# Mingtzge/PVE-MCC_for_unsignalized_intersection

Measured on AMD Instinct MI355X. Metric: env-steps/sec (vehicles x envs x steps/s) at 128 veh x 4096 envs, higher is better.
Workload: dtype f64

## Files before the change

pve-mcc_for_unsignalized_intersection_amd/csrc/pve_hip.hip:

```cpp
#include <hip/hip_runtime.h>
#include <mutex>
#include <new>

#include "pve_host.h"
#include "pve_tick_core.h"
#include "pve_tick_geo.h"
#include "pve_actor.h"

using namespace pve;

#ifdef PVE_AB_KNOBS
#define PVE_KNOB(name_) getenv(name_)
#else
#define PVE_KNOB(name_) ((const char *)nullptr)
#endif
#ifndef PVE_HOME_DEFAULT
#define PVE_HOME_DEFAULT 1
#endif

typedef __attribute__((address_space(4))) const char *KernargPtr;
#define PVE_PHASE_MARK(idx)                                                              \
    if (P.phase_cycles) {                                                                \
        unsigned long long now_ = wall_clock64();                                        \
        pc_[idx] = now_ - tprev_;                                                        \
        tprev_ = now_;                                                                   \
    }

__device__ __forceinline__ void lds_barrier() { __syncthreads(); }
template <int CAP>
__global__ __launch_bounds__(CAP) __attribute__((amdgpu_waves_per_eu(CAP == 128 ? 5 : 4, CAP == 128 ? 5 : 4))) void k_tick(const Const c_arg, const Params P_arg)
{
    KernargPtr ka0_ = (KernargPtr)__builtin_amdgcn_kernarg_segment_ptr();
    const PVE_AS4 Const &c = *(const PVE_AS4 Const *)ka0_;
    const PVE_AS4 Params &P = *(const PVE_AS4 Params *)(ka0_ + ((sizeof(Const) + 7) / 8 * 8));
    typedef Shared<CAP, false> ShT;
    __shared__ ShT sh;
    const int t = threadIdx.x;
    const int env = blockIdx.x;
    Regs r;
    typedef Tick<CAP, ShT> T;
    unsigned long long pc_[12] = {0, 0, 0, 0, 0, 0, 0, 0, 0, 0, 0, 0};
    unsigned long long tprev_ = P.phase_cycles ? wall_clock64() : 0ull;
    T::ph_load(c, P, env, t, sh, r);
    lds_barrier();
    PVE_PHASE_MARK(0)
    if (P.stop_phase == 0) return;
    T::ph_step1(c, P, env, t, sh, r);
    lds_barrier();
    PVE_PHASE_MARK(1)
    if (P.stop_phase == 1) return;
    T::ph_step2(c, t, sh, r);
    T::ph_lists_a(c, t, sh);
    lds_barrier();
    PVE_PHASE_MARK(2)
    if (P.stop_phase == 2) return;
    T::ph_step3(c, t, sh, r);
    T::ph_step3_publish(t, sh, r);
    T::ph_lists_b(t, sh);
    lds_barrier();
    PVE_PHASE_MARK(3)
    if (P.stop_phase == 3) return;
    T::ph_build(c, t, sh, r);
    lds_barrier();
    PVE_PHASE_MARK(4)
    if (P.stop_phase == 4) return;
    T::ph_rank(t, sh, env);
    lds_barrier();
    PVE_PHASE_MARK(5)
    if (P.stop_phase == 5) return;
    T::ph_scan(c, t, sh, r);
    PVE_PHASE_MARK(11)
    T::ph_reward(c, t, sh, r);
    lds_barrier();
    PVE_PHASE_MARK(6)
    if (P.stop_phase == 6) return;
    T::ph_effects(c, t, sh, r);
    lds_barrier();
    PVE_PHASE_MARK(7)
    if (P.stop_phase == 7) return;
    T::ph_prefetch_arrival(P, env, t, sh, r, NL);
    T::ph_lock(c, t, sh, r);
    lds_barrier();
    T::ph_lock2(t, sh, r);
    lds_barrier();
    PVE_PHASE_MARK(8)
    if (P.stop_phase == 8) return;
    T::ph_final(c, P, env, t, sh, r);
    PVE_PHASE_MARK(9)
    if (P.out.state_pre) {
        __threadfence_block();
        __syncthreads();
        if constexpr (CAP <= 128) {
            T::ph_state_publish(P.out, t, sh, r);
            __syncthreads();
            T::ph_state_coop(P, P.out, env, t, sh);
        } else T::ph_state(P, env, t, sh, r);
        PVE_PHASE_MARK(10)
    }
    if (P.phase_cycles && (t & 63) == 0) {
        unsigned long long *row = P.phase_cycles + ((size_t)env * (CAP / 64) + (t >> 6)) * 16;
#pragma unroll
        for (int k = 0; k < 12; k++) row[k] += pc_[k];
    }
}

template <int CAP>
__device__ __forceinline__ void rollout_actor(const unsigned char *packed, const float *aprm, double *act, const slot_t<CAP> *adsts,
                                              int n_ctl, const void *rows, bool obs_f32, size_t base, int t)
{
    const pve_v8h *A1 = (const pve_v8h *)(packed + AP_A1), *A2 = (const pve_v8h *)(packed + AP_A2);
    const int lane = t & 63, hf = lane >> 5, j = lane & 31;
    for (int tile = t >> 6; 32 * tile < n_ctl; tile += CAP / 64) {
        const int slot = adsts[32 * tile + j];
        const int srow = slot == SLOT_NONE<CAP> ? 0 : slot;
        float x[16];
        if (obs_f32) actor_fetch_env((const float *)rows + base * OBSW, srow, hf, x);
        else actor_fetch_env((const double *)rows + base * OBSW, srow, hf, x);
        const float a = actor_tile32(A1, A2, aprm, x, lane);
        if (lane < 32 && slot != SLOT_NONE<CAP>) act[slot] = (double)a;
    }
}

__device__ __forceinline__ void rollout_noise(const PVE_AS4 RolloutArgsNoisy &R, int env, int tick, Regs &r)
{
    const double sigma = R.noise.sigma;
    if (__builtin_expect(sigma != 0, 0)) {
        if (r.alive && (r.meta & M_CONTROL))
            r.act = r.act + sigma * action_noise_z(R.noise.seed, (int64_t)env + R.noise.env_offset, r.id, R.noise.tick0 + (uint32_t)tick);
    }
}

__device__ __forceinline__ double table_action(const double *table, int row, int table_ids, int id)
{
    const unsigned col = (unsigned)id < (unsigned)table_ids ? (unsigned)id : (unsigned)(table_ids - 1);
    return *(const double *)((const char *)(table + (size_t)row * (size_t)table_ids) + col * 8u);
}

#ifdef PVE_QUEUE_TRACE
#define Q_TRACE(R_) ((R_).q_trace)
#else
#define Q_TRACE(R_) ((unsigned long long *)nullptr)
#endif
__device__ __forceinline__ unsigned q_xcc_id()
{
    return __builtin_amdgcn_s_getreg((3 << 11) | (0 << 6) | 20) & 0xFu;
}
__device__ __forceinline__ unsigned q_load(const unsigned *p) { return __hip_atomic_load(p, __ATOMIC_RELAXED, __HIP_MEMORY_SCOPE_AGENT); }
__device__ __forceinline__ void q_store(unsigned *p, unsigned v) { __hip_atomic_store(p, v, __ATOMIC_RELAXED, __HIP_MEMORY_SCOPE_AGENT); }
__device__ __forceinline__ void q_dequeue(RolloutQueue *Q, int n_shards, int n_envs, int n_chunks, unsigned xcc, int &shard, int &probe,
                                          int &env, int &chunk)
{
    for (;;) {
        if (shard >= 0) {
            const unsigned es = (unsigned)(n_envs - shard + n_shards - 1) / (unsigned)n_shards;
            const unsigned i = __hip_atomic_fetch_add(&Q->s[shard].head, 1u, __ATOMIC_RELAXED, __HIP_MEMORY_SCOPE_AGENT);
            if (i < es * (unsigned)n_chunks) {
                const unsigned c = i / es;
                env = shard + (int)(i - c * es) * n_shards; chunk = (int)c;
                return;
            }
        }
        shard = -1;
        while (probe < n_shards) {
            const int cand = (int)((xcc + (unsigned)probe) % (unsigned)n_shards);
            probe++;
            if (cand >= n_envs) continue;
            unsigned seen = q_load(&Q->s[cand].owner);
            if (seen == 0u)
                __hip_atomic_compare_exchange_strong(&Q->s[cand].owner, &seen, xcc + 1u, __ATOMIC_RELAXED, __ATOMIC_RELAXED, __HIP_MEMORY_SCOPE_AGENT);
            if (seen != 0u && seen != xcc + 1u) continue;
            const unsigned es = (unsigned)(n_envs - cand + n_shards - 1) / (unsigned)n_shards;
            if (q_load(&Q->s[cand].head) >= es * (unsigned)n_chunks) continue;
            shard = cand;
            break;
        }
        if (shard < 0) { env = -1; chunk = 0; return; }
    }
}

__device__ __forceinline__ bool q_take(const PVE_AS4 RolloutArgs &R, int n_envs, int t0, int *q_word, int &env, int &chunk, int &k_base,
                                       int &n_ticks)
{
    RolloutQueue *Q = (RolloutQueue *)R.queue;
    unsigned *done = R.queue + sizeof(RolloutQueue) / 4;
    if (t0 == 0) {
        int shard = q_word[2], probe = q_word[3], e, ch;
        const unsigned long long tq0 = Q_TRACE(R) ? wall_clock64() : 0ull;
        q_dequeue(Q, R.n_shards, n_envs, R.n_full + R.n_taper, q_xcc_id(), shard, probe, e, ch);
        q_word[0] = e; q_word[1] = ch; q_word[2] = shard; q_word[3] = probe;
        const unsigned long long tq1 = Q_TRACE(R) ? wall_clock64() : 0ull;
        if (e >= 0)
            while ((int)(q_load(&done[e]) - (R.done_base + (unsigned)ch)) < 0) __builtin_amdgcn_s_sleep(8);
        if (Q_TRACE(R) && e >= 0) {
            unsigned long long *row = Q_TRACE(R) + ((size_t)ch * n_envs + e) * 8;
            row[0] = tq0; row[1] = tq1; row[2] = wall_clock64();
            row[6] = (unsigned long long)blockIdx.x | ((unsigned long long)q_xcc_id() << 32);
        }
    }
    __syncthreads();
    env = __builtin_amdgcn_readfirstlane(q_word[0]);
    chunk = __builtin_amdgcn_readfirstlane(q_word[1]);
    if (env < 0) return false;
    rollout_item(R, chunk, k_base, n_ticks);
    return true;
}
__device__ __forceinline__ void q_publish(const PVE_AS4 RolloutArgs &R, int n_envs, int t0, int env, int chunk)
{
    const unsigned long long tf0 = (Q_TRACE(R) && t0 == 0) ? wall_clock64() : 0ull;
    asm volatile("s_waitcnt vmcnt(0)" ::: "memory");
    __syncthreads();
    if (t0 == 0) q_store(R.queue + sizeof(RolloutQueue) / 4 + env, R.done_base + (unsigned)chunk + 1u);
    if (Q_TRACE(R) && t0 == 0) {
        unsigned long long *row = Q_TRACE(R) + ((size_t)chunk * n_envs + env) * 8;
        row[4] = tf0; row[5] = wall_clock64();
    }
}
__device__ __forceinline__ void q_leave(const PVE_AS4 RolloutArgs &R, int t0)
{
    RolloutQueue *Q = (RolloutQueue *)R.queue;
    if (t0 == 0) {
        const unsigned left = __hip_atomic_fetch_add(&Q->exits, 1u, __ATOMIC_RELAXED, __HIP_MEMORY_SCOPE_AGENT);
        if (left + 1u == gridDim.x) {
            for (int k = 0; k < QUEUE_MAX_SHARDS; k++) { q_store(&Q->s[k].head, 0u); q_store(&Q->s[k].owner, 0u); }
            q_store(&Q->exits, 0u);
        }
    }
}

template <int CAP, int WPE, bool PROF = false, bool ACT = false, bool TRAIN = false, bool IDT = false, bool PERS = false>
__global__ __launch_bounds__(CAP) __attribute__((amdgpu_waves_per_eu(WPE, WPE))) void k_rollout(const Const c_arg, const Params P_arg,
                                                                                               const typename rollout_args<ACT>::type R_arg)
{
    typedef typename rollout_args<ACT>::type RArgs;
    static_assert(!PERS || !PROF, "the persistent form has no phase-cycle diagnostics variant");
    static_assert(!(ACT && IDT), "one action source per variant");
    KernargPtr ka0_ = (KernargPtr)__builtin_amdgcn_kernarg_segment_ptr();
    constexpr size_t OFF_P = (sizeof(Const) + 7) / 8 * 8, OFF_R = OFF_P + (sizeof(Params) + 7) / 8 * 8;
    typedef Shared<CAP, (CAP == 128 && WPE == 4), (WPE == 5)> ShT;
    __shared__ ShT sh;
    __shared__ __attribute__((aligned(64))) float aprm[ACT ? PV_TOTAL : 1];
    __shared__ slot_t<CAP> adsts[ACT ? CAP : 1];
    __shared__ int q_word[4];
    int adst = -1;
    int t0_ = threadIdx.x;
    int env0_ = PERS ? 0 : blockIdx.x;
    int k_base_ = 0, chunk_ = 0;
    bool aprm_staged = false;
    if (CAP > 64) { if (__builtin_amdgcn_readfirstlane(t0_) < 64) __builtin_amdgcn_s_setprio(3); else if (WPE == 5) __builtin_amdgcn_s_setprio(2); }
    KernargPtr kav_ = ka0_;
    Regs r;
    FinCarry fc;
    typedef Tick<CAP, ShT> T;
    unsigned long long pc_[12] = {0, 0, 0, 0, 0, 0, 0, 0, 0, 0, 0, 0};
    unsigned long long tprev_ = PROF ? wall_clock64() : 0ull;
    const unsigned long long sclk0_ = PROF ? clock64() : 0ull, wclk0_ = tprev_;
#undef PVE_PHASE_MARK
#define PVE_PHASE_MARK(idx)                                                              \
    if (PROF) {                                                                          \
        unsigned long long now_ = wall_clock64();                                        \
        pc_[idx] += now_ - tprev_;                                                       \
        tprev_ = now_;                                                                   \
    }
    int pool_idx, n_ticks;
    if constexpr (PERS) { if (t0_ == 0) { q_word[2] = -1; q_word[3] = 0; } }
  for (;;) {
    {
        const PVE_AS4 Const &c = *(const PVE_AS4 Const *)ka0_;
        const PVE_AS4 Params &P = *(const PVE_AS4 Params *)(ka0_ + OFF_P);
        const PVE_AS4 RArgs &R = *(const PVE_AS4 RArgs *)(ka0_ + OFF_R);
        pool_idx = R.pool_tick0;
        n_ticks = R.n_ticks;
        const double *act0 = nullptr;
        if constexpr (PERS) {
            int e, ch, kb, nt;
            if (!q_take(R, P.n_envs, t0_, q_word, e, ch, kb, nt)) break;
            env0_ = e; chunk_ = ch; k_base_ = kb; n_ticks = nt;
            if (R.source == 1 || R.source == 3) pool_idx = (R.pool_tick0 + k_base_) % R.n_pool;
            if (R.source == 1) act0 = R.pool + (size_t)pool_idx * (size_t)P.n_envs * CAP;
        }
        bool act_handed = false;
        if constexpr (PERS && ACT) {
            act_handed = chunk_ > 0;
            if (act_handed) act0 = R.actor_actions;
        }
        if constexpr (ACT) if (!act_handed) {
            if (!PERS || !aprm_staged) {
                const float *gp = (const float *)(R.actor_packed + AP_PRM);
                for (int n = t0_; n < PV_TOTAL; n += CAP) aprm[n] = gp[n];
            }
            const int mt = P.i32[I_META][(size_t)env0_ * CAP + t0_];
            const bool cc = (mt & (M_ALIVE | M_CONTROL)) == (M_ALIVE | M_CONTROL);
            vote<CAP / 64>(sh.m_ctl, t0_, cc);
            adsts[t0_] = (slot_t<CAP>)SLOT_NONE<CAP>;
            lds_barrier();
            if (cc) adsts[mask_rank<CAP / 64>(sh.m_ctl, t0_)] = (slot_t<CAP>)t0_;
            const int nc = mask_count<CAP / 64>(sh.m_ctl);
            lds_barrier();
            rollout_actor<CAP>(R.actor_packed, aprm, sh.act_next, adsts, nc, R.actor_obs, P.obs_f32 != 0, (size_t)env0_ * CAP, t0_);
            lds_barrier();
        }
        if constexpr (PERS && ACT) {
            if (!aprm_staged && act_handed) {
                const float *gp = (const float *)(R.actor_packed + AP_PRM);
                for (int n = t0_; n < PV_TOTAL; n += CAP) aprm[n] = gp[n];
            }
            aprm_staged = true;
        }
        if constexpr (PERS) {
            T::template ph_load<true, ACT>(c, P, env0_, t0_, sh, r, act0, true);
            if (Q_TRACE(R) && t0_ == 0) Q_TRACE(R)[((size_t)chunk_ * P.n_envs + env0_) * 8 + 3] = wall_clock64();
        } else T::ph_load(c, P, env0_, t0_, sh, r);
        if constexpr (ACT) { if (!act_handed) r.act = sh.act_next[t0_]; }
        if constexpr (IDT) {
            r.act = r.alive ? table_action(R.pool, pool_idx, R.table_ids, r.id) : 0.0;
        }
        T::ph_home_store(t0_, sh, r);
    }
    double sp_act = 0;
    for (int k = 0; k < n_ticks; k++) {
        if constexpr (PERS) env0_ = __builtin_amdgcn_readfirstlane(env0_);
        asm volatile("" : "+s"(kav_), "+v"(t0_), "+s"(env0_));
        const KernargPtr ka = kav_;
        const int t = t0_, env = env0_;
#ifndef PVE_NO_RANGE_ASSUME
#ifdef PVE_ASSUME_ONE_WAVE_ONLY
        if constexpr (CAP == 64)
#endif
        __builtin_assume(t >= 0 && t < CAP);
#endif
        const PVE_AS4 Const &c = *(const PVE_AS4 Const *)ka;
        const PVE_AS4 Params &P = *(const PVE_AS4 Params *)(ka + OFF_P);
        const PVE_AS4 RArgs &R = *(const PVE_AS4 RArgs *)(ka + OFF_R);
        lds_barrier();
        PVE_PHASE_MARK(0)
        if constexpr (CAP == 64 && !PERS) {
            const int na = __builtin_amdgcn_readfirstlane(sh.hd.n_alive);
#ifndef PVE_NO_LOAD_PRIO
            if (na > 38) __builtin_amdgcn_s_setprio(3);
            else if (na > 32) __builtin_amdgcn_s_setprio(2);
            else if (na > 26) __builtin_amdgcn_s_setprio(1);
            else __builtin_amdgcn_s_setprio(0);
#endif
        }
        if (k > 0) T::ph_tick_init(c, t, sh, r);
        if constexpr (ACT) rollout_noise(R, env, k_base_ + k, r);
        T::ph_step1(c, P, env, t, sh, r);
        lds_barrier();
        PVE_PHASE_MARK(1)
        T::ph_step2(c, t, sh, r);
        T::ph_lists_a(c, t, sh);
        lds_barrier();
        PVE_PHASE_MARK(2)
        const bool last_tick = k + 1 == n_ticks;
        T::ph_step3(c, t, sh, r, last_tick);
        T::ph_step3_publish(t, sh, r);
        T::ph_lists_b(t, sh);
        lds_barrier();
        PVE_PHASE_MARK(3)
        if constexpr (ShT::HOME) {
            T::ph_build_prep(c, t, sh, r);
            T::ph_scan_init(r);
            if (__builtin_amdgcn_readfirstlane((int)sh.loff[NL]) <= ShT::POOL) {
                T::template ph_build_fill<false>(c, t, sh, r, 0, NL);
                lds_barrier();
                T::template ph_rank<false>(t, sh);
                lds_barrier();
                T::template ph_scan_lists<false>(c, t, sh, r, 0, NL);
            } else
            for (int d0 = 0, pass = 0; d0 < NL; pass++) {
                const int d1 = __builtin_amdgcn_readfirstlane(T::group_end(sh, d0));
                T::template ph_build_fill<true>(c, t, sh, r, d0, d1);
                lds_barrier();
                T::template ph_rank<true>(t, sh, pass, d0, d1);
                lds_barrier();
                T::template ph_scan_lists<true>(c, t, sh, r, d0, d1);
                d0 = d1;
                if (d0 < NL) lds_barrier();
            }
        } else {
        T::ph_build(c, t, sh, r);
        lds_barrier();
        PVE_PHASE_MARK(4)
        T::ph_rank(t, sh);
        lds_barrier();
        PVE_PHASE_MARK(5)
        T::ph_scan(c, t, sh, r);
        }
        PVE_PHASE_MARK(11)
        T::ph_reward(c, t, sh, r);
        lds_barrier();
        PVE_PHASE_MARK(6)
        int nx = -1;
        if (k + 1 < n_ticks) { pool_idx = (pool_idx + 1 == R.n_pool) ? 0 : pool_idx + 1; nx = pool_idx; }
        if constexpr (IDT) {
            int my_id = r.id;
            if constexpr (ShT::HOME) my_id = sh.h_id[t];
            r.act_nx = (nx >= 0 && r.alive) ? table_action(R.pool, nx, R.table_ids, my_id) : 0.0;
        } else T::ph_prefetch_action(P, R, env, t, nx, r);
        T::ph_effects(c, t, sh, r);
        lds_barrier();
        PVE_PHASE_MARK(7)
        T::ph_prefetch_arrival(P, env, t, sh, r, NL);
        bool sp_late = false;
        if constexpr (IDT) {
            const unsigned want = (unsigned)(sh.m_spawn[0] & 0xFFFull);
            sp_late = __builtin_popcount(want) > CAP - sh.hd.n_alive;
            sp_act = 0;
            if (t < NL && nx >= 0 && !sp_late && ((want >> t) & 1u))
                sp_act = table_action(R.pool, nx, R.table_ids, sh.hd.id_seq + __builtin_popcount(want & ((1u << t) - 1u)));
        }
        T::ph_lock(c, t, sh, r, last_tick);
        lds_barrier();
        T::ph_lock2(t, sh, r, last_tick);
        T::ph_keep_prefix(t, sh);
        lds_barrier();
        PVE_PHASE_MARK(8)
        if constexpr (!ACT && !IDT) { if (!(ShT::HOME && last_tick)) T::ph_park_action(t, sh, r); }
        const Outputs O = T::template tick_outputs<TRAIN>(P, R, k_base_ + k);
        if constexpr (ACT) {
            adst = -1;
            T::template ph_final<true>(c, P, O, env, t, sh, r, fc, true, &adst);
            adsts[t] = (slot_t<CAP>)(adst < 0 ? SLOT_NONE<CAP> : adst);
        } else T::template ph_final<true, !TRAIN>(c, P, O, env, t, sh, r, fc, k + 1 == n_ticks || (TRAIN && O.state_pre != nullptr));
        PVE_PHASE_MARK(9)
        if constexpr (IDT) {
            if (fc.new_slot >= 0) sh.act_next[fc.new_slot] = r.act_nx;
            if (sp_late) sp_act = (fc.sp_slot >= 0 && nx >= 0) ? table_action(R.pool, nx, R.table_ids, fc.sp_id) : 0.0;
        }
        HomeRegs hr;
        T::ph_home_take(t, sh, r, fc, hr);
        if (fc.still) {
            T::ph_stage_header(t, sh, fc);
            T::ph_carry_over(t, sh, r, fc);
        } else {
            lds_barrier();
            if constexpr (TRAIN) {
                if (O.state_pre) {
                    if constexpr (CAP <= 128) {
                        T::ph_state_publish(O, t, sh, r);
                        lds_barrier();
                        T::template ph_state_coop<PERS>(P, O, env, t, sh);
                    } else T::template ph_state<PERS>(P, O, env, t, sh, r);
                }
            }
            T::ph_stage(c, t, sh, r, fc);
            T::ph_home_put(t, sh, fc, hr);
            if constexpr (IDT) { if (fc.sp_slot >= 0) sh.act_next[fc.sp_slot] = sp_act; }
            if constexpr (ACT) {
                if (fc.sp_slot >= 0) sh.act_next[fc.sp_slot] = (double)aprm[PV_A0];
                const bool hand_on = PERS && k + 1 == n_ticks && chunk_ + 1 < R.n_full + R.n_taper;
                if (k + 1 < n_ticks || hand_on)
                    rollout_actor<CAP>(R.actor_packed, aprm, sh.act_next, adsts, fc.n_ctl, O.obs_post, P.obs_f32 != 0,
                                       (size_t)env * CAP, t);
                if (hand_on) {
                    lds_barrier();
                    R.actor_actions[(size_t)env * CAP + t] = sh.act_next[t];
                }
            }
            lds_barrier();
            if (k + 1 < n_ticks) T::ph_reload(t, sh, r);
        }
        PVE_PHASE_MARK(10)
    }
    {
        const PVE_AS4 Params &P = *(const PVE_AS4 Params *)(ka0_ + OFF_P);
        T::ph_flush(P, env0_, t0_, sh);
        if (PROF && P.phase_cycles && (t0_ & 63) == 0) {
            unsigned long long *row = P.phase_cycles + ((size_t)env0_ * (CAP / 64) + (t0_ >> 6)) * 16;
#pragma unroll
            for (int k = 0; k < 12; k++) row[k] += pc_[k];
            row[12] += clock64() - sclk0_; row[13] += wall_clock64() - wclk0_;
        }
    }
    if constexpr (PERS) {
        const PVE_AS4 RArgs &R = *(const PVE_AS4 RArgs *)(ka0_ + OFF_R);
        const PVE_AS4 Params &P = *(const PVE_AS4 Params *)(ka0_ + OFF_P);
        q_publish(R, P.n_envs, t0_, env0_, chunk_);
    } else break;
  }
    if constexpr (PERS) q_leave(*(const PVE_AS4 RArgs *)(ka0_ + OFF_R), t0_);
}

template <int CAP, bool PROF = false, bool FIX4 = false>
__global__ __launch_bounds__(CAP) __attribute__((amdgpu_waves_per_eu((CAP == 64 || FIX4) ? 4 : 5, (CAP == 64 || FIX4) ? 4 : 5))) void k_tick_geo(const GeoConst g_arg, const Params P_arg)
{
    KernargPtr ka0_ = (KernargPtr)__builtin_amdgcn_kernarg_segment_ptr();
    const PVE_AS4 GeoConst &g = *(const PVE_AS4 GeoConst *)ka0_;
    const PVE_AS4 Params &P = *(const PVE_AS4 Params *)(ka0_ + ((sizeof(GeoConst) + 7) / 8 * 8));
    __shared__ SharedGeo<CAP> sh;
    const int t = threadIdx.x;
    const int env = blockIdx.x;
    Regs r;
    typedef TickGeo<CAP> T;
    typedef Tick<CAP, SharedGeo<CAP>> B;
    unsigned long long pc_[12] = {0, 0, 0, 0, 0, 0, 0, 0, 0, 0, 0, 0};
    unsigned long long tprev_ = PROF ? wall_clock64() : 0ull;
#undef PVE_PHASE_MARK
#define PVE_PHASE_MARK(idx)                                                              \
    if (PROF) {                                                                          \
        unsigned long long now_ = wall_clock64();                                        \
        pc_[idx] = now_ - tprev_;                                                        \
        tprev_ = now_;                                                                   \
    }
    T::ph_load(g, P, env, t, sh, r);
    lds_barrier();
    PVE_PHASE_MARK(0)
    T::ph_step1(g, P, env, t, sh, r);
    lds_barrier();
    PVE_PHASE_MARK(1)
    B::ph_step2(g.base, t, sh, r);
    T::ph_order(t, sh, r);
    lds_barrier();
    PVE_PHASE_MARK(2)
    B::ph_step3(g.base, t, sh, r);
    B::ph_step3_publish(t, sh, r);
    T::ph_order2(t, sh, r);
    T::ph_pairs_mode(t, sh, P.geo_scan != 0);
    lds_barrier();
    PVE_PHASE_MARK(3)
    if (T::pairs_over(sh, P.geo_scan != 0)) {
        T::ph_pairs_count(g, t, sh, P.geo_scan != 0);
        lds_barrier();
        T::ph_pairs_exact(t, sh, P.geo_scan != 0);
        lds_barrier();
        T::ph_pairs_apply(t, sh);
        lds_barrier();
    }
    T::ph_pairs_fill(g, t, sh);
    lds_barrier();
    PVE_PHASE_MARK(4)
    T::ph_load_late(P, env, t, sh, r);
    if (FIX4) T::ph_fix_table(g, t, sh, r);
    T::ph_rank(t, sh, env);
    lds_barrier();
    PVE_PHASE_MARK(5)
    T::template ph_scan<FIX4>(g, t, sh, r);
    PVE_PHASE_MARK(11)
    T::ph_reward(g, t, sh, r);
    lds_barrier();
    PVE_PHASE_MARK(6)
    T::ph_effects(g, t, sh, r);
    lds_barrier();
    PVE_PHASE_MARK(7)
    B::ph_prefetch_arrival(P, env, t, sh, r, g.lane_num);
    B::ph_lock_slot(g.base, t, sh, r);
    if (P.out.state_pre) T::ph_state_order(t, sh, r);
    lds_barrier();
    B::ph_lock2_slot(t, sh, r);
    lds_barrier();
    PVE_PHASE_MARK(8)
    T::ph_final(g, P, env, t, sh, r);
    PVE_PHASE_MARK(9)
    if (P.out.state_pre) {
        __threadfence_block();
        __syncthreads();
        T::ph_state(P, env, t, sh, r);
    }
    if (PROF && P.phase_cycles && (t & 63) == 0) {
        unsigned long long *row = P.phase_cycles + ((size_t)env * (CAP / 64) + (t >> 6)) * 16;
#pragma unroll
        for (int k = 0; k < 12; k++) row[k] += pc_[k];
    }
}

template <int CAP, bool FIX4 = false, int WPE = 4, bool TRAIN = false, bool IDT = false, bool PERS = false, bool ACT = false>
__global__ __launch_bounds__(CAP) __attribute__((amdgpu_waves_per_eu(WPE, WPE))) void k_rollout_geo(const GeoConst g_arg, const Params P_arg,
                                                                                                const typename rollout_args<ACT>::type R_arg)
{
    typedef typename rollout_args<ACT>::type RArgs;
    static_assert(!(TRAIN && IDT), "lane_num 4 / 8: the table source without the training outputs");
    static_assert(!ACT || !IDT, "the closed loop of the geometry kernel: one action source");
    KernargPtr ka0_ = (KernargPtr)__builtin_amdgcn_kernarg_segment_ptr();
    constexpr size_t OFF_P = (sizeof(GeoConst) + 7) / 8 * 8, OFF_R = OFF_P + (sizeof(Params) + 7) / 8 * 8;
    __shared__ SharedGeo<CAP> sh;
    __shared__ __attribute__((aligned(64))) float aprm[ACT ? PV_TOTAL : 1];
    __shared__ uint8_t adsts[ACT ? CAP : 1];
    __shared__ int q_word[4];
    int t0_ = threadIdx.x;
    int env0_ = PERS ? 0 : blockIdx.x;
    int k_base_ = 0, chunk_ = 0;
    bool aprm_staged = false;
    KernargPtr kav_ = ka0_;
    Regs r;
    FinCarry fc;
    typedef TickGeo<CAP> T;
    typedef Tick<CAP, SharedGeo<CAP>> B;
    int pool_idx, n_ticks;
    if constexpr (PERS) { if (t0_ == 0) { q_word[2] = -1; q_word[3] = 0; } }
  for (;;) {
    {
        const PVE_AS4 GeoConst &g = *(const PVE_AS4 GeoConst *)ka0_;
        const PVE_AS4 Params &P = *(const PVE_AS4 Params *)(ka0_ + OFF_P);
        const PVE_AS4 RArgs &R = *(const PVE_AS4 RArgs *)(ka0_ + OFF_R);
        pool_idx = R.pool_tick0;
        n_ticks = R.n_ticks;
        const double *act0 = nullptr;
        if constexpr (PERS) {
            int e, ch, kb, nt;
            if (!q_take(R, P.n_envs, t0_, q_word, e, ch, kb, nt)) break;
            env0_ = e; chunk_ = ch; k_base_ = kb; n_ticks = nt;
            if (R.source == 1 || R.source == 3) pool_idx = (R.pool_tick0 + k_base_) % R.n_pool;
            if (R.source == 1) act0 = R.pool + (size_t)pool_idx * (size_t)P.n_envs * CAP;
        }
        bool act_handed = false;
        if constexpr (PERS && ACT) {
            act_handed = chunk_ > 0;
            if (act_handed) act0 = R.actor_actions;
        }
        if constexpr (ACT) if (!act_handed) {
            if (!PERS || !aprm_staged) {
                const float *gp = (const float *)(R.actor_packed + AP_PRM);
                for (int n = t0_; n < PV_TOTAL; n += CAP) aprm[n] = gp[n];
            }
            const int mt = P.i32[I_META][(size_t)env0_ * CAP + t0_];
            const bool cc = (mt & (M_ALIVE | M_CONTROL)) == (M_ALIVE | M_CONTROL);
            vote<CAP / 64>(sh.m_ctl, t0_, cc);
            adsts[t0_] = 255;
            lds_barrier();
            if (cc) adsts[mask_rank<CAP / 64>(sh.m_ctl, t0_)] = (uint8_t)t0_;
            const int nc = mask_count<CAP / 64>(sh.m_ctl);
            lds_barrier();
            rollout_actor<CAP>(R.actor_packed, aprm, sh.p, adsts, nc, R.actor_obs, P.obs_f32 != 0, (size_t)env0_ * CAP, t0_);
            lds_barrier();
        }
        if constexpr (PERS && ACT) {
            if (!aprm_staged && act_handed) {
                const float *gp = (const float *)(R.actor_packed + AP_PRM);
                for (int n = t0_; n < PV_TOTAL; n += CAP) aprm[n] = gp[n];
            }
            aprm_staged = true;
        }
        if constexpr (PERS) {
            T::template ph_load<true, ACT>(g, P, env0_, t0_, sh, r, act0, true);
            lds_barrier();
            T::template ph_load_late<true>(P, env0_, t0_, sh, r);
        } else {
        T::ph_load(g, P, env0_, t0_, sh, r);
        lds_barrier();
        T::ph_load_late(P, env0_, t0_, sh, r);
        }
        if constexpr (ACT) { if (!act_handed) r.act = sh.p[t0_]; }
        if constexpr (IDT) {
            const int idc = r.id < 0 ? 0 : (r.id < R.table_ids ? r.id : R.table_ids - 1);
            r.act = r.alive ? R.pool[(size_t)pool_idx * (size_t)R.table_ids + idc] : 0.0;
        }
    }
    double sp_act = 0;
    for (int k = 0; k < n_ticks; k++) {
        if constexpr (PERS) env0_ = __builtin_amdgcn_readfirstlane(env0_);
        asm volatile("" : "+s"(kav_), "+v"(t0_), "+s"(env0_));
        const KernargPtr ka = kav_;
        const int t = t0_, env = env0_;
#ifndef PVE_NO_RANGE_ASSUME
        __builtin_assume(t >= 0 && t < CAP);
#endif
        const PVE_AS4 GeoConst &g = *(const PVE_AS4 GeoConst *)ka;
        const PVE_AS4 Params &P = *(const PVE_AS4 Params *)(ka + OFF_P);
        const PVE_AS4 RArgs &R = *(const PVE_AS4 RArgs *)(ka + OFF_R);
        lds_barrier();
        if (k > 0) T::ph_tick_init(g, t, sh, r);
        if constexpr (ACT) rollout_noise(R, env, k_base_ + k, r);
        T::ph_step1(g, P, env, t, sh, r);
        lds_barrier();
        B::ph_step2(g.base, t, sh, r);
        T::ph_order(t, sh, r);
        lds_barrier();
        B::ph_step3(g.base, t, sh, r);
        B::ph_step3_publish(t, sh, r);
        T::ph_order2(t, sh, r);
        T::ph_pairs_mode(t, sh, P.geo_scan != 0);
        lds_barrier();
        if (T::pairs_over(sh, P.geo_scan != 0)) {
            T::ph_pairs_count(g, t, sh, P.geo_scan != 0);
            lds_barrier();
            T::ph_pairs_exact(t, sh, P.geo_scan != 0);
            lds_barrier();
            T::ph_pairs_apply(t, sh);
            lds_barrier();
        }
        T::ph_pairs_fill(g, t, sh);
        lds_barrier();
        if (FIX4) T::ph_fix_table(g, t, sh, r);
        T::ph_rank(t, sh);
        lds_barrier();
        T::template ph_scan<FIX4>(g, t, sh, r);
        T::ph_reward(g, t, sh, r);
        lds_barrier();
        int nx = -1;
        if (k + 1 < n_ticks) { pool_idx = (pool_idx + 1 == R.n_pool) ? 0 : pool_idx + 1; nx = pool_idx; }
        if constexpr (IDT) {
            const int idc = r.id < 0 ? 0 : (r.id < R.table_ids ? r.id : R.table_ids - 1);
            r.act_nx = (nx >= 0 && r.alive) ? R.pool[(size_t)nx * (size_t)R.table_ids + idc] : 0.0;
        } else B::ph_prefetch_action(P, R, env, t, nx, r);
        T::ph_effects(g, t, sh, r);
        T::ph_lists_clear(t, sh);
        lds_barrier();
        B::ph_prefetch_arrival(P, env, t, sh, r, g.lane_num);
        B::ph_lock_slot(g.base, t, sh, r);
        const Outputs O = B::template tick_outputs<TRAIN>(P, R, k_base_ + k);
        if (TRAIN && O.state_pre) T::ph_state_order(t, sh, r);
        lds_barrier();
        B::ph_lock2_slot(t, sh, r);
        lds_barrier();
        T::template ph_final<true>(g, P, O, env, t, sh, r, fc, ACT || k + 1 == n_ticks || (TRAIN && O.state_pre != nullptr));
        if constexpr (ACT) {
            if (t >= fc.n_ctl) adsts[t] = 255;
            if (r.alive && r.ctl) adsts[mask_rank<CAP / 64>(sh.m_ctl, t)] = (uint8_t)(fc.new_slot < 0 ? 255 : fc.new_slot);
        }
        if constexpr (IDT) {
            if (!fc.still && fc.new_slot >= 0) sh.p[fc.new_slot] = r.act_nx;
            sp_act = 0;
            if (fc.sp_slot >= 0 && nx >= 0) {
                const int idc = fc.sp_id < R.table_ids ? fc.sp_id : R.table_ids - 1;
                sp_act = R.pool[(size_t)nx * (size_t)R.table_ids + idc];
            }
        }
        if (fc.still) {
            T::ph_carry_over(t, sh, r, fc);
        } else {
            lds_barrier();
            if (TRAIN && O.state_pre) T::template ph_state<PERS>(P, O, env, t, sh, r);
            T::ph_stage(g, t, sh, r, fc);
            if constexpr (IDT) { if (fc.sp_slot >= 0) sh.p[fc.sp_slot] = sp_act; }
            if constexpr (ACT) {
                if (fc.sp_slot >= 0) sh.p[fc.sp_slot] = (double)aprm[PV_A0];
                const bool hand_on = PERS && k + 1 == n_ticks && chunk_ + 1 < R.n_full + R.n_taper;
                if (k + 1 < n_ticks || hand_on)
                    rollout_actor<CAP>(R.actor_packed, aprm, sh.p, adsts, fc.n_ctl, O.obs_post, P.obs_f32 != 0, (size_t)env * CAP, t);
                if (hand_on) {
                    lds_barrier();
                    R.actor_actions[(size_t)env * CAP + t] = sh.p[t];
                }
            }
            lds_barrier();
            if (k + 1 < n_ticks) {
                T::ph_reload(t, sh, r);
                if constexpr (IDT || ACT) r.act = sh.p[t];
            }
        }
    }
    {
        const PVE_AS4 Params &P = *(const PVE_AS4 Params *)(ka0_ + OFF_P);
        B::ph_flush(P, env0_, t0_, sh);
    }
    if constexpr (PERS) {
        const PVE_AS4 RArgs &R = *(const PVE_AS4 RArgs *)(ka0_ + OFF_R);
        const PVE_AS4 Params &P = *(const PVE_AS4 Params *)(ka0_ + OFF_P);
        q_publish(R, P.n_envs, t0_, env0_, chunk_);
    } else break;
  }
    if constexpr (PERS) q_leave(*(const PVE_AS4 RArgs *)(ka0_ + OFF_R), t0_);
}

#if defined(PVE_PROBE_ONE) || defined(PVE_PROBE_GEO)
#ifdef PVE_PROBE_ONE
template <int CAP, int WPE, bool PROF = false, bool ACT = false, bool... REST> struct probe_one_act { static constexpr bool value = ACT; };
template __global__ void k_rollout<PVE_PROBE_ONE>(const Const, const Params, const rollout_args<probe_one_act<PVE_PROBE_ONE>::value>::type);
#endif
#ifdef PVE_PROBE_GEO
template <int CAP, bool FIX4 = false, int WPE = 4, bool TRAIN = false, bool IDT = false, bool PERS = false, bool ACT = false> struct probe_geo_act { static constexpr bool value = ACT; };
template __global__ void k_rollout_geo<PVE_PROBE_GEO>(const GeoConst, const Params, const rollout_args<probe_geo_act<PVE_PROBE_GEO>::value>::type);
#endif
#else
template <int CAP>
__global__ __launch_bounds__(64) void k_reset_geo(const GeoConst g_arg, const Params P_arg, int cap_ticks)
{
    KernargPtr kar_ = (KernargPtr)__builtin_amdgcn_kernarg_segment_ptr();
    const PVE_AS4 GeoConst &g = *(const PVE_AS4 GeoConst *)kar_;
    const PVE_AS4 Params &P = *(const PVE_AS4 Params *)(kar_ + ((sizeof(GeoConst) + 7) / 8 * 8));
    const int env = blockIdx.x * blockDim.x + threadIdx.x;
    if (env < P.n_envs) reset_env_geo<CAP>(g, P, env, cap_ticks);
}

template <int CAP>
__global__ __launch_bounds__(CAP) void k_compact(const Params P_arg)
{
    const PVE_AS4 Params &P = *(const PVE_AS4 Params *)(KernargPtr)__builtin_amdgcn_kernarg_segment_ptr();
    __shared__ Shared<CAP> sh;
    const int t = threadIdx.x;
    const int env = blockIdx.x;
    CRegs r;
    Tick<CAP>::ph_c_load(P, env, t, sh, r);
    __syncthreads();
    Tick<CAP>::ph_c_store(P, env, t, sh, r);
}

template <int CAP>
__global__ __launch_bounds__(CAP) void k_probe(const Params P, int *sink)
{
    const size_t g = (size_t)blockIdx.x * CAP + threadIdx.x;
    double a = P.f64[F_P][g] + P.f64[F_V][g] + P.f64[F_A][g] + P.f64[F_JERK_SUM][g] + P.f64[F_VIR_DIS][g] +
               P.f64[F_CLOSER_P][g];
    int b = P.i32[I_ID][g] + P.i32[I_SEQ][g] + P.i32[I_VNUM][g] + P.i32[I_STEP][g] + P.i32[I_COUNT][g] +
            P.i32[I_META][g];
    unsigned long long m = __ballot(a + (double)b == 12345.678);
    if (threadIdx.x == 0) sink[blockIdx.x] = (int)m;
}

template <int CAP>
__global__ __launch_bounds__(64) void k_reset(const Const c_arg, const Params P_arg, int cap_ticks)
{
    KernargPtr kar_ = (KernargPtr)__builtin_amdgcn_kernarg_segment_ptr();
    const PVE_AS4 Const &c = *(const PVE_AS4 Const *)kar_;
    const PVE_AS4 Params &P = *(const PVE_AS4 Params *)(kar_ + ((sizeof(Const) + 7) / 8 * 8));
    const int env = blockIdx.x * blockDim.x + threadIdx.x;
    if (env < P.n_envs) reset_env<CAP>(c, P, env, cap_ticks);
}

static std::string hip_err(const char *what, hipError_t e)
{
    return std::string(what) + ": " + hipGetErrorString(e);
}

template <typename K> static hipError_t resident_blocks(int *nb, K kernel, int threads)
{
    hipError_t e = hipOccupancyMaxActiveBlocksPerMultiprocessor(nb, kernel, threads, 0);
    if (e != hipSuccess) return e;
    hipFuncAttributes fa;
    e = hipFuncGetAttributes(&fa, (const void *)kernel);
    if (e != hipSuccess) return e;
    if (fa.sharedSizeBytes > 0) {
        const int granules = (int)((fa.sharedSizeBytes + 1279) / 1280), by_lds = 128 / granules;
        if (by_lds > 0 && by_lds < *nb) *nb = by_lds;
    }
    return hipSuccess;
}

struct OccCache {
    static constexpr int MAX_DEV = 64;
    std::mutex mu;
    int wgs[MAX_DEV][4][3] = {};
    int n_cu[MAX_DEV] = {};
    template <typename Q>
    long long resident(int family, int cap, Q query, std::string &err)
    {
        int dev = 0;
        if (hipGetDevice(&dev) != hipSuccess) { err = "hipGetDevice failed"; return -1; }
        const int ci = cap == 64 ? 0 : (cap == 128 ? 1 : 2);
        std::lock_guard<std::mutex> lock(mu);
        const bool cached = dev >= 0 && dev < MAX_DEV && wgs[dev][family][ci] > 0;
        int nb = cached ? wgs[dev][family][ci] : 0, cus = cached ? n_cu[dev] : 0;
        if (!cached) {
            hipDeviceProp_t prop;
            const hipError_t e = query(&nb);
            if (e != hipSuccess || nb <= 0 || hipGetDeviceProperties(&prop, dev) != hipSuccess) {
                err = std::string("occupancy query of the persistent roll-out: ") + hipGetErrorString(e);
                return -1;
            }
            cus = prop.multiProcessorCount;
            if (dev >= 0 && dev < MAX_DEV) { wgs[dev][family][ci] = nb; n_cu[dev] = cus; }
        }
        return (long long)nb * cus;
    }
};
static OccCache g_occ;

struct Backend {
    static constexpr int max_capacity = 256;
    static int bad_cap(int cap, std::string &err)
    {
        err = "no kernel for capacity " + std::to_string(cap);
        return -1;
    }
    static int set_device(int dev, std::string &err)
    {
        int n = 0;
        hipError_t e = hipGetDeviceCount(&n);
        if (e != hipSuccess || n <= 0) { err = "no HIP device visible (libpveenv.so needs an AMD GPU; there is no CPU fallback)"; return -1; }
        if (dev < 0 || dev >= n) { err = "device_id out of range"; return -1; }
        return 0;
    }
    static int enter_device(int dev)
    {
        int prev = -1;
        if (hipGetDevice(&prev) != hipSuccess) prev = -1;
        if (prev != dev) (void)hipSetDevice(dev);
        return prev;
    }
    static void leave_device(int prev)
    {
        int cur = -1;
        if (prev >= 0 && hipGetDevice(&cur) == hipSuccess && cur != prev) (void)hipSetDevice(prev);
    }
    static void *dmalloc(size_t n)
    {
        void *p = nullptr;
        if (hipMalloc(&p, n) != hipSuccess) return nullptr;
        return p;
    }
    static void dfree(void *p) { (void)hipFree(p); }
    static int memset0(void *p, size_t n, void *stream)
    {
        return hipMemsetAsync(p, 0, n, (hipStream_t)stream) == hipSuccess ? 0 : -1;
    }
    static int n_xcc(int dev)
    {
        int v = 0;
        if (hipDeviceGetAttribute(&v, hipDeviceAttributeNumberOfXccs, dev) != hipSuccess || v <= 0) v = 8;
        return v > QUEUE_MAX_SHARDS ? QUEUE_MAX_SHARDS : v;
    }
    static int d2h(void *dst, const void *src, size_t n, void *stream)
// ... 279 lines not shown
```

pve-mcc_for_unsignalized_intersection_amd/csrc/pve_types.h:

```cpp
#pragma once
#include <stdint.h>
#include <stddef.h>

#if defined(__HIPCC__)
#include <hip/hip_runtime.h>
#define PVE_HD __host__ __device__ __forceinline__
#else
#define PVE_HD inline
#endif

namespace pve {

constexpr int NL = 12;
constexpr int ND = 16;
constexpr int MAXK = 8;
constexpr int OBSW = 28;
constexpr int NNB = 6;

constexpr int M_CONTROL = 0x1, M_FINISH = 0x2, M_DONE = 0x4, M_LOCK = 0x8;
constexpr int M_LOCKA_POS = 0x10, M_LOCKA_NEG = 0x20;
constexpr int M_DEL = 0x40;
constexpr int M_ALIVE = 0x80;
constexpr int M_COLL_SHIFT = 8, M_COLL_MASK = 0xFFFF;
constexpr int M_INT_SHIFT = 24, M_INT_MASK = 0x3;
constexpr int M_LANE_SHIFT = 26, M_LANE_MASK = 0xF;

constexpr int MODE_FUSED = 0;
constexpr int MODE_SCENE = 1;
constexpr int MODE_COMPACT = 2;

struct Const {
    double deltaT, dt2;
    double vm, vM, am, aM, v0;
    double abs_am, two_abs_am;
    double inv_abs_am, inv_two_abs_am;
    double aM_minus_am;
    double inv_dt, inv_span;
    double collision_thr, lock_mean_thr;
    double exit_p;
    double cw;
    double inbox[3];
    double spawn_p[3];
    double vdA[2][4], vdB[2][4], vdC[2][4];
    double rot_cos[4], rot_sin[4];
    double arc_k;
    int8_t l2l[NL][4];
    int8_t l2l_inv[NL][4];
};

struct EnvHeader {
    double current_time;
    double sum_reward, sum_jerk;
    double next_arr[NL];
    long long alive_steps, ctl_steps, ticks;
    int32_t n_alive;
    int32_t lane_start[NL + 1];
    int32_t veh_rec[NL];
    int32_t id_seq, passed, passed_step_total;
    int32_t head_valid;
    int32_t head_lane[ND], head_j[ND];
    int32_t collided, locks, overflow;
    int32_t intention_re;
};

enum { F_P = 0, F_V, F_A, F_JERK, F_JERK_SUM, F_VIR_DIS, F_CLOSER_P, NF64 };
enum { I_ID = 0, I_SEQ, I_VNUM, I_STEP, I_COUNT, I_META, I_HDR, NI32 };

struct GeoTab {
    double vd[4][MAXK][4];
    double inbox[4];
    int8_t pos[ND][ND];
    int8_t lst[ND][12];
    uint16_t mroutes[ND];
    uint16_t lroutes[ND];
    uint16_t ninv[ND];
    int8_t opp[ND];
    int8_t dir_lane[ND], dir_index[ND];
    int8_t nl[ND];
    int8_t dty[ND];
};

struct GeoConst {
    Const base;
    int32_t lane_num, dir_num, tmod, RL;
    double H;
    double fix_d, fix_hi, fix_lo;
    int8_t l2l[ND][MAXK];
    int8_t direction[NL][4];
    int8_t turn[NL];
    int8_t pad_[4];
    unsigned long long turn_pk, dir_pk[3];
    GeoTab tab;
};

struct Outputs {
    double *obs_post, *obs_pre, *state_pre;
    const double *obs_prev_post;
    double *reward;
    int32_t *flags, *lanej, *nbr, *new_slot, *env_out;
};

struct Params {
    EnvHeader *headers;
    double *f64[NF64];
    int32_t *i32[NI32];
    const double *actions;
    const double *arrivals;
    long long arr_env_stride;
    int32_t rows;
    int32_t n_envs;
    int32_t mode;
    int32_t mask_uncontrolled;
    int32_t obs_f32;
    int32_t geo_scan;
    const int32_t *choice;
    long long choice_env_stride;
    unsigned long long *phase_cycles;
    int32_t stop_phase;
    Outputs out;
};

struct ActionNoise {
    double sigma;
    uint64_t seed;
    int64_t env_offset;
    uint32_t tick0;
    uint32_t pad_;
};

struct RolloutArgs {
    const double *pool;
    const unsigned char *actor_packed;
    const void *actor_obs;
    const void *prev_rows;
    int32_t n_ticks, source, n_pool, pool_tick0, trajectory;
    int32_t table_ids;
    int32_t exact_f32;
    unsigned *queue;
    int32_t call_ticks;
    int32_t n_full, n_taper;
    uint8_t taper[8];
    int32_t n_shards;
    uint32_t done_base;
    double *actor_actions;
    unsigned long long *q_trace;
};
struct RolloutArgsNoisy : RolloutArgs {
    ActionNoise noise;
};
template <bool ACT> struct rollout_args { typedef RolloutArgs type; };
template <> struct rollout_args<true> { typedef RolloutArgsNoisy type; };

template <typename RA>
PVE_HD void rollout_item(const RA &R, int chunk, int &k_base, int &n_ticks)
{
    k_base = (chunk < R.n_full ? chunk : R.n_full) * R.n_ticks;
    for (int q = 0; q < chunk - R.n_full; q++) k_base += R.taper[q];
    n_ticks = chunk < R.n_full ? R.n_ticks : (int)R.taper[chunk - R.n_full];
}

constexpr int QUEUE_MAX_SHARDS = 16;
struct RolloutQueue {
    struct Shard {
        unsigned head;
        unsigned owner;
        unsigned pad_[30];
    } s[QUEUE_MAX_SHARDS];
    unsigned exits;
    unsigned pad_[31];
};

inline size_t align_up(size_t x, size_t a) { return (x + a - 1) / a * a; }

constexpr size_t ACTOR_FLAT_BYTES = 25600, ACTOR_PACKED_BYTES = 26880;

struct Layout {
    size_t off_headers, off_f64[NF64], off_i32[NI32], off_actor_flat, off_actor_packed, off_queue, total;
};

inline Layout make_layout(int n_envs, int cap)
{
    Layout L;
    size_t o = 0;
    L.off_headers = o; o = align_up(o + sizeof(EnvHeader) * (size_t)n_envs, 256);
    for (int k = 0; k < NF64; k++) { L.off_f64[k] = o; o = align_up(o + 8 * (size_t)n_envs * cap, 256); }
    for (int k = 0; k < NI32; k++) { L.off_i32[k] = o; o = align_up(o + 4 * (size_t)n_envs * cap, 256); }
    L.off_actor_flat = o; o = align_up(o + ACTOR_FLAT_BYTES, 256);
    L.off_actor_packed = o; o = align_up(o + ACTOR_PACKED_BYTES, 256);
    L.off_queue = o; o = align_up(o + sizeof(RolloutQueue) + 4 * (size_t)n_envs, 256);
    L.total = o;
    return L;
}

}
```

Baseline: 22.98 billion.

## Split queue shards into sub-heads and prefetch next work item before flush

```diff
diff --git a/pve-mcc_for_unsignalized_intersection_amd/csrc/pve_hip.hip b/pve-mcc_for_unsignalized_intersection_amd/csrc/pve_hip.hip
--- a/pve-mcc_for_unsignalized_intersection_amd/csrc/pve_hip.hip
+++ b/pve-mcc_for_unsignalized_intersection_amd/csrc/pve_hip.hip
@@ -147,17 +147,38 @@
 }
 __device__ __forceinline__ unsigned q_load(const unsigned *p) { return __hip_atomic_load(p, __ATOMIC_RELAXED, __HIP_MEMORY_SCOPE_AGENT); }
 __device__ __forceinline__ void q_store(unsigned *p, unsigned v) { __hip_atomic_store(p, v, __ATOMIC_RELAXED, __HIP_MEMORY_SCOPE_AGENT); }
-__device__ __forceinline__ void q_dequeue(RolloutQueue *Q, int n_shards, int n_envs, int n_chunks, unsigned xcc, int &shard, int &probe,
-                                          int &env, int &chunk)
-{
+__device__ __forceinline__ const PVE_AS4 RolloutArgs &q_args(const PVE_AS4 RolloutArgs &R_in)
+{
+    const PVE_AS4 RolloutArgs *p = &R_in;
+    asm volatile("" : "+s"(p));
+    return *p;
+}
+__device__ __forceinline__ unsigned *q_head(RolloutQueue *Q, int shard, int sub)
+{
+    return sub == 0 ? &Q->s[shard].head : &Q->sub[shard][sub - 1].head;
+}
+constexpr int Q_WARM = 1 << 24, Q_PRE = 1 << 25;
+__device__ __forceinline__ void q_dequeue(RolloutQueue *Q, int n_shards, int n_envs, int n_chunks, unsigned xcc, int &shard, int &st,
+                                          unsigned pre, int &env, int &chunk)
+{
+    int probe = st & 0xFF, sub = (st >> 8) & 0xFF, nsub = (st >> 16) & 0xFF;
+    bool warm = (st & Q_WARM) != 0, have_pre = (st & Q_PRE) != 0;
     for (;;) {
         if (shard >= 0) {
-            const unsigned es = (unsigned)(n_envs - shard + n_shards - 1) / (unsigned)n_shards;
-            const unsigned i = __hip_atomic_fetch_add(&Q->s[shard].head, 1u, __ATOMIC_RELAXED, __HIP_MEMORY_SCOPE_AGENT);
-            if (i < es * (unsigned)n_chunks) {
-                const unsigned c = i / es;
-                env = shard + (int)(i - c * es) * n_shards; chunk = (int)c;
-                return;
+            const unsigned es = queue_shard_envs(n_envs, n_shards, shard);
+            while (nsub < QUEUE_SUBS) {
+                const unsigned m = queue_sub_envs(es, sub), lim = m * (unsigned)n_chunks;
+                unsigned *head = q_head(Q, shard, sub);
+                unsigned i = lim;
+                if (have_pre) { i = pre; have_pre = false; }
+                else if (lim != 0u && (warm || (nsub == 0 && probe <= 1) || q_load(head) < lim))
+                    i = __hip_atomic_fetch_add(head, 1u, __ATOMIC_RELAXED, __HIP_MEMORY_SCOPE_AGENT);
+                if (i < lim) {
+                    env = queue_item_env(n_shards, shard, sub, m, i, chunk);
+                    st = probe | (sub << 8) | (nsub << 16) | Q_WARM;
+                    return;
+                }
+                warm = false; nsub++; sub = (sub + 1) % QUEUE_SUBS;
             }
         }
         shard = -1;
@@ -169,25 +190,39 @@
             if (seen == 0u)
                 __hip_atomic_compare_exchange_strong(&Q->s[cand].owner, &seen, xcc + 1u, __ATOMIC_RELAXED, __ATOMIC_RELAXED, __HIP_MEMORY_SCOPE_AGENT);
             if (seen != 0u && seen != xcc + 1u) continue;
-            const unsigned es = (unsigned)(n_envs - cand + n_shards - 1) / (unsigned)n_shards;
-            if (q_load(&Q->s[cand].head) >= es * (unsigned)n_chunks) continue;
-            shard = cand;
+            shard = cand; sub = (int)((blockIdx.x / (unsigned)n_shards) % QUEUE_SUBS); nsub = 0; warm = false;
             break;
         }
-        if (shard < 0) { env = -1; chunk = 0; return; }
-    }
-}
-
-__device__ __forceinline__ bool q_take(const PVE_AS4 RolloutArgs &R, int n_envs, int t0, int *q_word, int &env, int &chunk, int &k_base,
+        if (shard < 0) { env = -1; chunk = 0; st = probe | (QUEUE_SUBS << 16); return; }
+    }
+}
+__device__ __forceinline__ unsigned q_pretake(const PVE_AS4 RolloutArgs &R_in, int t0, int *q_word)
+{
+    const PVE_AS4 RolloutArgs &R = q_args(R_in);
+    unsigned pre = 0u;
+#ifndef PVE_NO_PRETAKE
+    if (t0 == 0) {
+        const int shard = q_word[2], st = q_word[3];
+        if (shard >= 0 && (st & Q_WARM)) {
+            pre = __hip_atomic_fetch_add(q_head((RolloutQueue *)R.queue, shard, (st >> 8) & 0xFF), 1u, __ATOMIC_RELAXED, __HIP_MEMORY_SCOPE_AGENT);
+            q_word[3] = st | Q_PRE;
+        }
+    }
+#endif
+    return pre;
+}
+
+__device__ __forceinline__ bool q_take(const PVE_AS4 RolloutArgs &R_in, int n_envs, int t0, int *q_word, int &env, int &chunk, int &k_base,
                                        int &n_ticks)
 {
+    const PVE_AS4 RolloutArgs &R = q_args(R_in);
     RolloutQueue *Q = (RolloutQueue *)R.queue;
     unsigned *done = R.queue + sizeof(RolloutQueue) / 4;
     if (t0 == 0) {
-        int shard = q_word[2], probe = q_word[3], e, ch;
+        int shard = q_word[2], st = q_word[3], e, ch;
         const unsigned long long tq0 = Q_TRACE(R) ? wall_clock64() : 0ull;
-        q_dequeue(Q, R.n_shards, n_envs, R.n_full + R.n_taper, q_xcc_id(), shard, probe, e, ch);
-        q_word[0] = e; q_word[1] = ch; q_word[2] = shard; q_word[3] = probe;
+        q_dequeue(Q, R.n_shards, n_envs, R.n_full + R.n_taper, q_xcc_id(), shard, st, (unsigned)q_word[0], e, ch);
+        q_word[0] = e; q_word[1] = ch; q_word[2] = shard; q_word[3] = st;
         const unsigned long long tq1 = Q_TRACE(R) ? wall_clock64() : 0ull;
         if (e >= 0)
             while ((int)(q_load(&done[e]) - (R.done_base + (unsigned)ch)) < 0) __builtin_amdgcn_s_sleep(8);
@@ -204,10 +239,12 @@
     rollout_item(R, chunk, k_base, n_ticks);
     return true;
 }
-__device__ __forceinline__ void q_publish(const PVE_AS4 RolloutArgs &R, int n_envs, int t0, int env, int chunk)
-{
+__device__ __forceinline__ void q_publish(const PVE_AS4 RolloutArgs &R_in, int n_envs, int t0, int env, int chunk, int *q_word, unsigned pre)
+{
+    const PVE_AS4 RolloutArgs &R = q_args(R_in);
     const unsigned long long tf0 = (Q_TRACE(R) && t0 == 0) ? wall_clock64() : 0ull;
     asm volatile("s_waitcnt vmcnt(0)" ::: "memory");
+    if (t0 == 0) q_word[0] = (int)pre;
     __syncthreads();
     if (t0 == 0) q_store(R.queue + sizeof(RolloutQueue) / 4 + env, R.done_base + (unsigned)chunk + 1u);
     if (Q_TRACE(R) && t0 == 0) {
@@ -215,13 +252,17 @@
         row[4] = tf0; row[5] = wall_clock64();
     }
 }
-__device__ __forceinline__ void q_leave(const PVE_AS4 RolloutArgs &R, int t0)
-{
+__device__ __forceinline__ void q_leave(const PVE_AS4 RolloutArgs &R_in, int t0)
+{
+    const PVE_AS4 RolloutArgs &R = q_args(R_in);
     RolloutQueue *Q = (RolloutQueue *)R.queue;
     if (t0 == 0) {
         const unsigned left = __hip_atomic_fetch_add(&Q->exits, 1u, __ATOMIC_RELAXED, __HIP_MEMORY_SCOPE_AGENT);
         if (left + 1u == gridDim.x) {
-            for (int k = 0; k < QUEUE_MAX_SHARDS; k++) { q_store(&Q->s[k].head, 0u); q_store(&Q->s[k].owner, 0u); }
+            for (int k = 0; k < R.n_shards; k++) {
+                for (int q = 0; q < QUEUE_SUBS; q++) q_store(q_head(Q, k, q), 0u);
+                q_store(&Q->s[k].owner, 0u);
+            }
             q_store(&Q->exits, 0u);
         }
     }
@@ -462,8 +503,10 @@
         }
         PVE_PHASE_MARK(10)
     }
+    unsigned q_pre = 0u;
     {
         const PVE_AS4 Params &P = *(const PVE_AS4 Params *)(ka0_ + OFF_P);
+        if constexpr (PERS) q_pre = q_pretake(*(const PVE_AS4 RArgs *)(ka0_ + OFF_R), t0_, q_word);
         T::ph_flush(P, env0_, t0_, sh);
         if (PROF && P.phase_cycles && (t0_ & 63) == 0) {
             unsigned long long *row = P.phase_cycles + ((size_t)env0_ * (CAP / 64) + (t0_ >> 6)) * 16;
@@ -475,7 +518,7 @@
     if constexpr (PERS) {
         const PVE_AS4 RArgs &R = *(const PVE_AS4 RArgs *)(ka0_ + OFF_R);
         const PVE_AS4 Params &P = *(const PVE_AS4 Params *)(ka0_ + OFF_P);
-        q_publish(R, P.n_envs, t0_, env0_, chunk_);
+        q_publish(R, P.n_envs, t0_, env0_, chunk_, q_word, q_pre);
     } else break;
   }
     if constexpr (PERS) q_leave(*(const PVE_AS4 RArgs *)(ka0_ + OFF_R), t0_);
@@ -739,14 +782,16 @@
             }
         }
     }
+    unsigned q_pre = 0u;
     {
         const PVE_AS4 Params &P = *(const PVE_AS4 Params *)(ka0_ + OFF_P);
+        if constexpr (PERS) q_pre = q_pretake(*(const PVE_AS4 RArgs *)(ka0_ + OFF_R), t0_, q_word);
         B::ph_flush(P, env0_, t0_, sh);
     }
     if constexpr (PERS) {
         const PVE_AS4 RArgs &R = *(const PVE_AS4 RArgs *)(ka0_ + OFF_R);
         const PVE_AS4 Params &P = *(const PVE_AS4 Params *)(ka0_ + OFF_P);
-        q_publish(R, P.n_envs, t0_, env0_, chunk_);
+        q_publish(R, P.n_envs, t0_, env0_, chunk_, q_word, q_pre);
     } else break;
   }
     if constexpr (PERS) q_leave(*(const PVE_AS4 RArgs *)(ka0_ + OFF_R), t0_);
diff --git a/pve-mcc_for_unsignalized_intersection_amd/csrc/pve_types.h b/pve-mcc_for_unsignalized_intersection_amd/csrc/pve_types.h
--- a/pve-mcc_for_unsignalized_intersection_amd/csrc/pve_types.h
+++ b/pve-mcc_for_unsignalized_intersection_amd/csrc/pve_types.h
@@ -160,6 +160,7 @@
 }
 
 constexpr int QUEUE_MAX_SHARDS = 16;
+constexpr int QUEUE_SUBS = 8;
 struct RolloutQueue {
     struct Shard {
         unsigned head;
@@ -168,7 +169,26 @@
     } s[QUEUE_MAX_SHARDS];
     unsigned exits;
     unsigned pad_[31];
-};
+    struct Sub {
+        unsigned head;
+        unsigned pad_[31];
+    } sub[QUEUE_MAX_SHARDS][QUEUE_SUBS - 1];
+};
+
+PVE_HD unsigned queue_shard_envs(int n_envs, int n_shards, int shard)
+{
+    return shard < n_envs ? (unsigned)(n_envs - shard + n_shards - 1) / (unsigned)n_shards : 0u;
+}
+PVE_HD unsigned queue_sub_envs(unsigned shard_envs, int sub)
+{
+    return (unsigned)sub < shard_envs ? (shard_envs - (unsigned)sub + QUEUE_SUBS - 1) / QUEUE_SUBS : 0u;
+}
+PVE_HD int queue_item_env(int n_shards, int shard, int sub, unsigned sub_envs, unsigned item, int &chunk)
+{
+    const unsigned c = item / sub_envs;
+    chunk = (int)c;
+    return shard + (sub + (int)(item - c * sub_envs) * QUEUE_SUBS) * n_shards;
+}
 
 inline size_t align_up(size_t x, size_t a) { return (x + a - 1) / a * a; }
 
```

After: 22.95 billion (median of 3 runs). No clear change (-0.1%).
